# caojiezhang/CiaoSR

Hardware: AMD Instinct MI355X
Metric: HR Mpix/s (RDN-CiaoSR x4, LocalImplicitSR forward_test) (higher is better)
Workload: dtype f32; 1 GPU; C3: RDN-CiaoSR (c64b16) x4, LR 1356x2040 -> 5424x8160 (DIV2K-shaped 2K LR), tiled inference: 117 tiles of 192x192 (overlap 32), random-init weights, fp32; scale=4, tiles=117, parallelism=tile-shard x1

## Files before the change

### ciaosr_amd/_lib.py

```python
import ctypes as C
import os

_HERE = os.path.dirname(os.path.abspath(__file__))
LIB_PATH = os.environ.get('CIAOSR_HIP_LIB') or os.path.join(_HERE, 'csrc', 'libciaosr_hip.so')
MAX_LAYERS = 8

ACT_NONE, ACT_RELU, ACT_PRELU, ACT_GELU, ACT_SIN, ACT_COS = 0, 1, 2, 3, 4, 5


class CiaoSRHipError(RuntimeError):
    pass


class MlpT(C.Structure):
    _fields_ = [('n_layers', C.c_int), ('act', C.c_int), ('in_dim', C.c_int), ('width', C.c_int * MAX_LAYERS),
                ('weight', C.c_void_p * MAX_LAYERS), ('ld', C.c_int * MAX_LAYERS),
                ('bias', C.c_void_p * MAX_LAYERS), ('frag', C.c_void_p * MAX_LAYERS),
                ('frag16', C.c_void_p * MAX_LAYERS), ('frag16_lo', C.c_void_p * MAX_LAYERS)]


class HeadWeightsT(C.Structure):
    _fields_ = [('channels', C.c_int), ('nonlocal_channels', C.c_int), ('nonlocal_max_scale', C.c_int), ('local_size', C.c_int),
                ('no_unfold', C.c_int),
                ('softmax_scale', C.c_float), ('q', MlpT), ('k', MlpT), ('v', MlpT), ('k_out_wino', C.c_void_p), ('k_out_wino4', C.c_void_p),
                ('chain16', C.c_void_p), ('chain16_pairs', C.c_void_p)]


class HeadSceneT(C.Structure):
    _fields_ = [(n, C.c_int) for n in ('magic', 'H', 'W', 'C', 'Cn', 'D', 'Dv', 'J', 'q_plan', 'precision', 'route',
                                       'off_u', 'off_tk', 'off_tv', 'off_g', 'total')]


class CsAttnWeightsT(C.Structure):
    _fields_ = [('channels', C.c_int), ('scale', C.c_int),
                ('w_match1', C.c_void_p), ('b_match1', C.c_void_p), ('slope_match1', C.c_float),
                ('w_match2', C.c_void_p), ('b_match2', C.c_void_p), ('slope_match2', C.c_float),
                ('w_assembly', C.c_void_p), ('b_assembly', C.c_void_p), ('slope_assembly', C.c_float),
                ('w_down', C.c_void_p), ('b_down', C.c_void_p), ('w_down_masked', C.c_void_p),
                ('escape_nan', C.c_float), ('softmax_scale', C.c_float)]


class OptionsT(C.Structure):
    _fields_ = [('head_route', C.c_int), ('csa_composed_min', C.c_int), ('dense_min_tiles', C.c_int),
                ('scatter_small_max', C.c_int), ('kv_rows', C.c_int), ('decode_rows', C.c_int), ('bf16_single', C.c_int),
                ('dense_direct', C.c_int), ('csa_scores_gemm', C.c_int), ('csa_attn_tile128', C.c_int), ('query_grid_w', C.c_int), ('f16_pairs', C.c_int),
                ('csa_attn_v16', C.c_int), ('edsr_resident', C.c_int), ('swin_h16', C.c_int), ('csa_block_mb', C.c_int)]


HEAD_STAGED, HEAD_NO_LOGIT_TABLE, HEAD_TABLE_GEMM, HEAD_WIDE_WG, HEAD_TABLE_WINO2, HEAD_NO_CHAIN, HEAD_NO_DECODE_CHAIN = 1, 2, 4, 8, 16, 32, 64


class ConvT(C.Structure):
    _fields_ = [('weight', C.c_void_p), ('bias', C.c_void_p), ('cin', C.c_int), ('cout', C.c_int), ('ksize', C.c_int),
                ('frag16', C.c_void_p), ('frag16_lo', C.c_void_p), ('frag', C.c_void_p), ('frag_wino', C.c_void_p),
                ('frag_wino4', C.c_void_p)]


class RdnWeightsT(C.Structure):
    _fields_ = [('mid_channels', C.c_int), ('growth', C.c_int), ('num_blocks', C.c_int), ('num_layers', C.c_int),
                ('sfe1', ConvT), ('sfe2', ConvT), ('gff0', ConvT), ('gff1', ConvT),
                ('dense', C.POINTER(ConvT)), ('lff', C.POINTER(ConvT)),
                ('scatter_weight', C.POINTER(C.c_void_p)), ('scatter_bias', C.c_void_p),
                ('scatter_frag', C.POINTER(C.c_void_p))]


class SwinBlockT(C.Structure):
    _fields_ = [(n, C.c_void_p) for n in ('ln1_w', 'ln1_b', 'qkv_w', 'qkv_b', 'bias', 'proj_w', 'proj_b', 'ln2_w', 'ln2_b',
                                           'fc1_w', 'fc1_b', 'fc2_w', 'fc2_b')] + [('shift', C.c_int), ('mask', C.c_void_p)] + \
               [(n, C.c_void_p) for n in ('qkv_w16', 'proj_w16', 'fc1_w16', 'fc2_w16')]


class SwinirWeightsT(C.Structure):
    _fields_ = [('embed_dim', C.c_int), ('num_heads', C.c_int), ('window_size', C.c_int), ('hidden', C.c_int),
                ('num_groups', C.c_int), ('depth', C.c_int), ('conv_first', ConvT), ('conv_after_body', ConvT),
                ('pe_norm_w', C.c_void_p), ('pe_norm_b', C.c_void_p), ('norm_w', C.c_void_p), ('norm_b', C.c_void_p),
                ('blocks', C.POINTER(SwinBlockT)), ('group_conv', C.POINTER(ConvT))]


class EdsrWeightsT(C.Structure):
    _fields_ = [('mid_channels', C.c_int), ('num_blocks', C.c_int), ('res_scale', C.c_float),
                ('conv_first', ConvT), ('conv_after_body', ConvT),
                ('conv1', C.POINTER(ConvT)), ('conv2', C.POINTER(ConvT))]


_P, _I, _F, _S = C.c_void_p, C.c_int, C.c_float, C.c_size_t
_O = C.POINTER(OptionsT)

SIGNATURES = {
    'ciaosr_version': (_I, []),
    'ciaosr_error_string': (C.c_char_p, [_I]),
    'ciaosr_sizeof': (_S, [C.c_char_p]),
    'ciaosr_prof_enable': (_I, [_I]),
    'ciaosr_prof_filter': (_I, [C.c_char_p]),
    'ciaosr_prof_reset': (_I, []),
    'ciaosr_prof_collect': (_I, []),
    'ciaosr_prof_get': (_I, [C.c_char_p, C.POINTER(C.c_double), C.POINTER(C.c_long)]),
    'ciaosr_prof_names': (_I, [C.c_char_p, _I]),
    'ciaosr_nchw_to_hwc_f32': (_I, [_P, _P, _I, _I, _I, _I, _P]),
    'ciaosr_hwc_to_nchw_f32': (_I, [_P, _I, _P, _I, _I, _I, _P]),
    'ciaosr_gemm_f32': (_I, [_P, _I, _P, _I, _I, _P, _I, _P, _I, _I, _I, _F, _I, _F, _P]),
    'ciaosr_patch_rows_f32': (_I, [_P, _I, _I, _I, _I, _I, _I, _I, _I, _I, _P, _I, _I, _F, _P]),
    'ciaosr_cs_attn_workspace_bytes': (_S, [_I, _I, _I]),
    'ciaosr_cs_attn_workspace_bytes_scale': (_S, [_I, _I, _I, _I]),
    'ciaosr_cs_attn_workspace_bytes_opt': (_S, [_I, _I, _I, _I, _O]),
    'ciaosr_cs_attn_block_rows': (_I, [_I, _I, _I, _I, _I, _O]),
    'ciaosr_cs_attn_f32': (_I, [_P, _I, _I, _I, C.POINTER(CsAttnWeightsT), _P, _I, _O, _P, _S, _P]),
    'ciaosr_cs_attn_bf16': (_I, [_P, _I, _I, _I, C.POINTER(CsAttnWeightsT), _P, _I, _O, _P, _S, _P]),
    'ciaosr_make_coord_cell_f32': (_I, [_P, _P, _I, _I, _P]),
    'ciaosr_make_coord_cell_window_f32': (_I, [_P, _P, _I, _I, _I, _I, _I, _I, C.POINTER(_I), _P]),
    'ciaosr_fragment_floats': (_S, [_I, _I]),
    'ciaosr_pack_fragments_f32': (_I, [_P, _I, _I, _I, _P, _P]),
    'ciaosr_cs_attn_f16': (_I, [_P, _I, _I, _I, C.POINTER(CsAttnWeightsT), _P, _I, _O, _P, _S, _P]),
    'ciaosr_fragment_bf16_bytes': (_S, [_I, _I]),
    'ciaosr_fragment_f16_bytes': (_S, [_I, _I]),
    'ciaosr_pack_fragments_f16': (_I, [_P, _I, _I, _I, _P, _P]),
    'ciaosr_pack_fragments_bf16': (_I, [_P, _I, _I, _I, _P, _P]),
    'ciaosr_pack_fragments_bf16_lo': (_I, [_P, _I, _I, _I, _P, _P]),
    'ciaosr_pack_fragments_f16_lo': (_I, [_P, _I, _I, _I, _P, _P]),
    'ciaosr_pack_fragments_bf16_pair': (_I, [_P, _I, _I, _I, _P, _P, _P]),
    'ciaosr_pack_fragments_f16_pair': (_I, [_P, _I, _I, _I, _P, _P, _P]),
    'ciaosr_pack_conv3x3_f32': (_I, [_P, _S, _S, _S, _S, _I, _I, _P, _P, _P, _P]),
    'ciaosr_head_chain_bytes': (_S, [C.POINTER(HeadWeightsT), _I]),
    'ciaosr_pack_head_chain_bf16': (_I, [C.POINTER(HeadWeightsT), _I, _P, _P]),
    'ciaosr_pack_head_chain_f16': (_I, [C.POINTER(HeadWeightsT), _I, _P, _P]),
    'ciaosr_head_indices_f32': (_I, [_P, _P, _I, _I, _I, _I, _I, _P, _P, _P, _P]),
    'ciaosr_local_attention_f32': (_I, [_P, _I, _I, _I, _P, _P, _P, _I, _P, _I, _P, _I, _I, _I, _F, _P]),
    'ciaosr_local_attention_bf16': (_I, [_P, _I, _I, _I, _P, _P, _P, _I, _P, _I, _P, _I, _I, _I, _F, _P]),
    'ciaosr_local_attention_f16': (_I, [_P, _I, _I, _I, _P, _P, _P, _I, _P, _I, _P, _I, _I, _I, _F, _P]),
    'ciaosr_gather_rows_f32': (_I, [_P, _I, _I, _I, _P, _P, _I, _I, _I, _I, _I, _P, _I, _P, _I, _P, _I, _P, _P, _P]),
    'ciaosr_mlp_workspace_bytes': (_S, [C.POINTER(MlpT), _I]),
    'ciaosr_mlp_forward_f32': (_I, [_P, _I, C.POINTER(MlpT), _I, _I, _P, _I, _P, _S, _P]),
    'ciaosr_mlp_workspace_bytes_16': (_S, [C.POINTER(MlpT), _I]),
    'ciaosr_mlp_forward_bf16': (_I, [_P, _I, C.POINTER(MlpT), _I, _P, _I, _P, _S, _P]),
    'ciaosr_mlp_forward_f16': (_I, [_P, _I, C.POINTER(MlpT), _I, _P, _I, _P, _S, _P]),
    'ciaosr_decode_residual_f32': (_I, [_P, _I, _I, _P, _I, _P, _P, _P, _I, _I, _I, _P, _P]),
    'ciaosr_head_workspace_bytes': (_S, [_I, _I, C.POINTER(HeadWeightsT), _I]),
    'ciaosr_head_workspace_bytes_opt': (_S, [_I, _I, C.POINTER(HeadWeightsT), _I, _O]),
    'ciaosr_head_forward_f32': (_I, [_P, _I, _I, C.POINTER(HeadWeightsT), C.POINTER(CsAttnWeightsT), _P, _P, _P,
                                     _I, _I, _P, _O, _P, _S, _P]),
    'ciaosr_head_forward_bf16': (_I, [_P, _I, _I, C.POINTER(HeadWeightsT), C.POINTER(CsAttnWeightsT), _P, _P, _P,
                                      _I, _I, _P, _O, _P, _S, _P]),
    'ciaosr_head_forward_f16': (_I, [_P, _I, _I, C.POINTER(HeadWeightsT), C.POINTER(CsAttnWeightsT), _P, _P, _P,
                                      _I, _I, _P, _O, _P, _S, _P]),
    'ciaosr_head_route_code': (_I, [_I, _I, C.POINTER(HeadWeightsT), _I, _I, _O]),
    'ciaosr_head_scene_bytes': (_S, [_I, _I, C.POINTER(HeadWeightsT), _I, _O]),
    'ciaosr_head_prepare_workspace_bytes': (_S, [_I, _I, C.POINTER(HeadWeightsT), _I, _O]),
    'ciaosr_head_query_workspace_bytes': (_S, [C.POINTER(HeadSceneT), C.POINTER(HeadWeightsT), _I, _O]),
    'ciaosr_head_query_flag_offset': (_I, [C.POINTER(HeadSceneT), C.POINTER(HeadWeightsT), _I, _O, C.POINTER(_S)]),
    **{'ciaosr_head_prepare_' + sfx: (_I, [_P, _I, _I, C.POINTER(HeadWeightsT), C.POINTER(CsAttnWeightsT), _I, _O, _P, _S,
                                          C.POINTER(HeadSceneT), _P, _S, _P]) for sfx in ('f32', 'bf16', 'f16')},
    **{'ciaosr_head_query_' + sfx: (_I, [_P, _S, C.POINTER(HeadSceneT), C.POINTER(HeadWeightsT), _P, _P, _P, _I, _I, _P, _O, _P, _S, _P])
       for sfx in ('f32', 'bf16', 'f16')},
    'ciaosr_rdn_workspace_bytes': (_S, [_I, _I, C.POINTER(RdnWeightsT)]),
    'ciaosr_rdn_forward_f32': (_I, [_P, _I, _I, C.POINTER(RdnWeightsT), _P, _O, _P, _S, _P]),
    'ciaosr_rdn_forward_bf16': (_I, [_P, _I, _I, C.POINTER(RdnWeightsT), _P, _O, _P, _S, _P]),
    'ciaosr_rdn_forward_f16': (_I, [_P, _I, _I, C.POINTER(RdnWeightsT), _P, _O, _P, _S, _P]),
    'ciaosr_rdn_workspace_bytes_batch': (_S, [_I, _I, _I, C.POINTER(RdnWeightsT)]),
    'ciaosr_rdn_forward_batch_f32': (_I, [_P, _I, _I, _I, C.POINTER(RdnWeightsT), _P, _O, _P, _S, _P]),
    'ciaosr_rdn_forward_batch_bf16': (_I, [_P, _I, _I, _I, C.POINTER(RdnWeightsT), _P, _O, _P, _S, _P]),
    'ciaosr_rdn_forward_batch_f16': (_I, [_P, _I, _I, _I, C.POINTER(RdnWeightsT), _P, _O, _P, _S, _P]),
    'ciaosr_edsr_workspace_bytes': (_S, [_I, _I, C.POINTER(EdsrWeightsT)]),
    'ciaosr_edsr_forward_f32': (_I, [_P, _I, _I, C.POINTER(EdsrWeightsT), _P, _P, _S, _P]),
    'ciaosr_edsr_workspace_bytes_batch': (_S, [_I, _I, _I, C.POINTER(EdsrWeightsT), _O]),
    'ciaosr_edsr_route_code': (_I, [_I, _I, _I, C.POINTER(EdsrWeightsT), _O]),
    'ciaosr_edsr_forward_batch_f32': (_I, [_P, _I, _I, _I, C.POINTER(EdsrWeightsT), _P, _O, _P, _S, _P]),
    'ciaosr_swinir_workspace_bytes': (_S, [_I, _I, C.POINTER(SwinirWeightsT)]),
    'ciaosr_swinir_forward_f32': (_I, [_P, _I, _I, C.POINTER(SwinirWeightsT), _P, _P, _S, _P]),
    'ciaosr_swinir_workspace_bytes_batch_f16': (_S, [_I, _I, _I, C.POINTER(SwinirWeightsT)]),
    'ciaosr_swinir_forward_batch_f16': (_I, [_P, _I, _I, _I, C.POINTER(SwinirWeightsT), _P, _O, _P, _S, _P]),
    'ciaosr_normalize_f32': (_I, [_P, _P, _I, _I, C.POINTER(_F), C.POINTER(_F), _P]),
    'ciaosr_denorm_clamp_f32': (_I, [_P, _P, _I, _I, C.POINTER(_F), C.POINTER(_F), _P]),
    'ciaosr_tile_blend_f32': (_I, [_P, _P, _I, _I, _P, _I, _I, _I, _I, _P]),
    'ciaosr_tile_finalize_f32': (_I, [_P, _P, _P, _I, _I, _P]),
    'ciaosr_view_block_queries': (_I, []),
    'ciaosr_view_workspace_bytes': (_S, [_I, _I, _I]),
    'ciaosr_view_coord_cell_f32': (_I, [_P, _P, C.POINTER(C.c_double), _I, _I, C.POINTER(_I), _P]),
    'ciaosr_view_count_i32': (_I, [C.POINTER(C.c_double), _I, _I, _P, _I, _P, _P, _S, _P]),
    'ciaosr_view_count_many_max_views': (_I, []),
    'ciaosr_view_many_workspace_bytes': (_S, [C.POINTER(_I), _I, _I]),
    'ciaosr_view_many_workspace_offset': (_S, [C.POINTER(_I), _I, _I, _I]),
# ... 57 lines not shown
```

### ciaosr_amd/csrc/dense_wino4_f32.hip

```cpp
#include "ops.h"
#include <type_traits>

namespace ciaosr {

typedef float f32x16 __attribute__((ext_vector_type(16)));
typedef float f32x4 __attribute__((ext_vector_type(4)));
typedef float f32x2 __attribute__((ext_vector_type(2)));
typedef int i32x4 __attribute__((ext_vector_type(4)));

constexpr int W4TH = 16, W4TW = 32;
constexpr int W4PH = W4TH + 2, W4PW = W4TW + 2;
constexpr int W4NP = W4PH * W4PW;
constexpr int W4PIECES = (2 * W4NP + 63) / 64;
constexpr int W4PATCH = W4PIECES * 1024;
constexpr int W4VROW = 32;
constexpr int W4VPOS = 32 * W4VROW;
constexpr int W4V = 36 * W4VPOS;
constexpr int W4V0 = 2 * W4PATCH;
constexpr size_t kWino4Xch = 4 * 8 * 4 * 64 * 16;
constexpr size_t kWino4Loop = 2 * (size_t)W4PATCH + 2 * (size_t)W4V;
constexpr size_t kWino4Lds = kWino4Loop > kWino4Xch ? kWino4Loop : kWino4Xch;
constexpr unsigned kOobW4 = 0xFFFFFFF0u;

struct DenseWino4P {
    float* x; int ldx;
    unsigned x_bytes;
    int H, W, tiles_x;
    int groups;
    const float4* wf;
    int nj; long pos_stride;
    const float* bias;
    int col_out;
    float* out; unsigned out_bytes;
    int ld_out; unsigned out_img_bytes;
    unsigned wf_block_bytes;
};

struct W4Slot { int vfrag, window, w2, dma, wnext; };
constexpr W4Slot w4_slot_plan(int r3, int slot) {
    W4Slot s = {-1, -1, -1, -1, -1};
    if (r3 < 2 && slot % 4 == 0) s.vfrag = slot / 4;
    if (r3 < 2 && slot % 2 == 1) s.window = 12 * r3 + slot / 2;
    if (r3 == 0 && slot < 6) s.w2 = slot;
    if (r3 == 0 && slot >= 6 && slot % 4 == 2) s.dma = (slot - 6) / 4;
    if (r3 == 1 && slot % 4 == 2) s.wnext = slot / 4;
    if (r3 == 2 && slot < 18) {
        if (slot % 3 == 2) s.wnext = 6 + slot / 3;
        else s.window = 24 + 2 * (slot / 3) + slot % 3;
    }
    return s;
}

#define W4_BT(x0, x1, x2, x3, x4, x5, y0, y1, y2, y3, y4, y5)                          \
    do {                                                                               \
        const float t1_ = __builtin_fmaf(-4.f, x2, x4), t2_ = __builtin_fmaf(-4.f, x1, x3); \
        const float t3_ = x4 - x2, t4_ = x3 - x1;                                      \
        y0 = __builtin_fmaf(4.f, x0, __builtin_fmaf(-5.f, x2, x4));                   \
        y1 = t1_ + t2_;                                                                \
        y2 = t1_ - t2_;                                                                \
        y3 = __builtin_fmaf(2.f, t4_, t3_);                                            \
        y4 = __builtin_fmaf(-2.f, t4_, t3_);                                           \
        y5 = __builtin_fmaf(4.f, x1, __builtin_fmaf(-5.f, x3, x5));                   \
    } while (0)

#ifdef CIAOSR_PROBE
__device__ unsigned long long g_w4probe[1024 * 8];
#define W4PROBE(slot) do { if (threadIdx.x == 0 && blockIdx.y == 0 && blockIdx.x < 1024) g_w4probe[blockIdx.x * 8 + (slot)] = __builtin_readcyclecounter(); } while (0)
#define W4PROBE_ADD(slot, t0) do { w4acc##slot += __builtin_readcyclecounter() - (t0); } while (0)
#else
#define W4PROBE(slot) do { } while (0)
#define W4PROBE_ADD(slot, t0) do { } while (0)
#endif

template <bool TABLE>
__global__ __launch_bounds__(256) void dense_wino4_f32_kernel(DenseWino4P p) {
    extern __shared__ __attribute__((aligned(16))) unsigned char lds4[];
    W4PROBE(0);
#ifdef CIAOSR_PROBE
    unsigned long long w4acc5 = 0, w4acc6 = 0;
#endif
    const int t = threadIdx.x, lane = t & 63, w = __builtin_amdgcn_readfirstlane(t >> 6), li = lane & 31, lh = lane >> 5;
    const int nt = w & 1, h = w >> 1;
    const int ty0 = (blockIdx.x / p.tiles_x) * W4TH, tx0 = (blockIdx.x % p.tiles_x) * W4TW;
    const int img = blockIdx.y;
    const unsigned img_off = (unsigned)((size_t)img * p.H * p.W * p.ldx * 4);
    const unsigned lds0 = (unsigned)(size_t)(__attribute__((address_space(3))) unsigned char*)lds4;

    constexpr int W4DS = W4PIECES / 4;
    unsigned goff[W4DS];
#pragma unroll
    for (int s = 0; s < W4DS; ++s) {
        const int qs = 64 * (w + 4 * s) + lane;
        const int q = qs ^ (((qs >> 3) & 3) << 1);
        const int P = q >> 1, half = q & 1;
        const int py = P / W4PW, px = P - py * W4PW;
        const int gy = ty0 - 1 + py, gx = tx0 - 1 + px;
        const bool ok = P < W4NP && gy >= 0 && gy < p.H && gx >= 0 && gx < p.W;
        goff[s] = ok ? (img_off + (unsigned)(gy * p.W + gx) * (unsigned)p.ldx * 4u + (unsigned)half * 16u) : kOobW4;
    }
    const int rot = p.groups > 1 ? (int)(blockIdx.x % (unsigned)p.groups) : 0;
    auto phys = [&](int g) -> int { const int x = g + rot; return x >= p.groups ? x - p.groups : x; };
    const i32x4 desc = {(int)(unsigned)(size_t)p.x, (int)(((size_t)p.x >> 32) & 0xFFFFu), (int)p.x_bytes, 0x00020000};
    const int N = 8 * p.groups;
    auto step_ch = [&](int n) -> int { return 64 * phys(n >> 3) + 8 * (n & 7); };
    auto dma_patch = [&](int n) {
        const unsigned soff = __builtin_amdgcn_readfirstlane((unsigned)step_ch(n) * 4u);
#pragma unroll
        for (int s = 0; s < W4DS; ++s) {
            const unsigned dst = __builtin_amdgcn_readfirstlane(lds0 + (unsigned)((n & 1) * W4PATCH) + 1024u * (unsigned)(w + 4 * s));
            unsigned keep;
            asm volatile("s_mov_b32 %0, m0\n\ts_mov_b32 m0, %2\n\ts_nop 0\n\tbuffer_load_dwordx4 %1, %3, %4 offen lds\n\ts_mov_b32 m0, %0"
                         : "=&s"(keep) : "v"(goff[s]), "s"(dst), "s"(desc), "s"(soff) : "memory");
        }
    };

    const int tch = t & 7, ttile = t >> 3;
    const int ttyw = ttile >> 3, ttxw = ttile & 7;
    int ty[4][4];
    {
        const int P0 = 4 * W4PW * ttyw + 4 * ttxw;
        const int k0 = (P0 >> 2) & 3;
        const int tbase = 32 * P0 + 16 * (tch >> 2) + 4 * (tch & 3);
#pragma unroll
        for (int m = 0; m < 4; ++m)
#pragma unroll
            for (int c = 0; c < 4; ++c) ty[m][c] = tbase + 32 * (m ^ ((k0 + c) & 3));
    }
    const int tvoff = ((2 * ttile + (tch >> 2)) ^ ((ttile >> 3) & 1)) * 16 + (tch & 3) * 4;

    const i32x4 wdesc = {(int)(unsigned)(size_t)p.wf, (int)(((size_t)p.wf >> 32) & 0xFFFFu), (int)0xFFFFFFFFu, 0x00020000};
    const unsigned lane16 = (unsigned)lane * 16u;
    const unsigned pos_bytes = (unsigned)p.pos_stride * 16u;
    auto wload = [&](f32x4& dst, int pp, int n) __attribute__((always_inline)) {
        const unsigned so = __builtin_amdgcn_readfirstlane((unsigned)(18 * h + pp) * pos_bytes + (unsigned)(nt * p.nj + (step_ch(n) >> 3)) * 1024u +
                                                           (TABLE ? (unsigned)blockIdx.z * p.wf_block_bytes : 0u));
        asm volatile("buffer_load_dwordx4 %0, %1, %2, %3 offen" : "=v"(dst) : "v"(lane16), "s"(wdesc), "s"(so) : "memory");
    };

    dma_patch(0);
    if (N > 1) dma_patch(1);
    f32x4 wr[18];
#pragma unroll
    for (int pp = 0; pp < 12; ++pp) wload(wr[pp], pp, 0);
    __builtin_amdgcn_sched_barrier(0);
    f32x16 acc[18];
#pragma unroll
    for (int pp = 0; pp < 18; ++pp)
#pragma unroll
        for (int e = 0; e < 16; ++e) acc[pp][e] = 0.f;
    asm volatile("s_waitcnt vmcnt(12)" ::: "memory");
    __builtin_amdgcn_s_barrier();
    __builtin_amdgcn_sched_barrier(0);

    W4PROBE(1);
    float dn[36];
    auto patch_value = [&](int n, int o36) __attribute__((always_inline)) -> float {
        const int a = o36 / 6, b = o36 - 6 * a, o = W4PW * a + b;
        return *reinterpret_cast<const float*>(lds4 + (n & 1) * W4PATCH + ty[o & 3][(o >> 2) & 3] + 32 * (o & ~3));
    };
#pragma unroll
    for (int o36 = 0; o36 < 36; ++o36) dn[o36] = patch_value(0, o36);
    const int vfo = ((2 * li + lh) ^ ((li >> 3) & 1)) * 16;
#pragma unroll 1
    for (int n = 0; n < N; ++n) {
#ifdef CIAOSR_PROBE
        const unsigned long long tstep = __builtin_readcyclecounter();
#endif
        {
            unsigned char* vb = lds4 + W4V0 + (n & 1) * W4V + tvoff;
            float d[6][6];
#pragma unroll
            for (int a = 0; a < 6; ++a)
#pragma unroll
                for (int b = 0; b < 6; ++b) d[a][b] = dn[6 * a + b];
            float r[6][6];
#pragma unroll
            for (int bp = 0; bp < 3; ++bp) {
                f32x2 x[6], y[6];
#pragma unroll
                for (int a = 0; a < 6; ++a) x[a] = f32x2{d[a][2 * bp], d[a][2 * bp + 1]};
                const f32x2 t1 = __builtin_elementwise_fma(f32x2{-4.f, -4.f}, x[2], x[4]), t2 = __builtin_elementwise_fma(f32x2{-4.f, -4.f}, x[1], x[3]);
                const f32x2 t3 = x[4] - x[2], t4 = x[3] - x[1];
                y[0] = __builtin_elementwise_fma(f32x2{4.f, 4.f}, x[0], __builtin_elementwise_fma(f32x2{-5.f, -5.f}, x[2], x[4]));
                y[1] = t1 + t2;
                y[2] = t1 - t2;
                y[3] = __builtin_elementwise_fma(f32x2{2.f, 2.f}, t4, t3);
                y[4] = __builtin_elementwise_fma(f32x2{-2.f, -2.f}, t4, t3);
                y[5] = __builtin_elementwise_fma(f32x2{4.f, 4.f}, x[1], __builtin_elementwise_fma(f32x2{-5.f, -5.f}, x[3], x[5]));
#pragma unroll
                for (int i = 0; i < 6; ++i) { r[i][2 * bp] = y[i][0]; r[i][2 * bp + 1] = y[i][1]; }
            }
#pragma unroll
            for (int i = 0; i < 6; ++i) {
                float v0, v1, v2, v3, v4, v5;
                W4_BT(r[i][0], r[i][1], r[i][2], r[i][3], r[i][4], r[i][5], v0, v1, v2, v3, v4, v5);
                *reinterpret_cast<float*>(vb + (6 * i + 0) * W4VPOS) = v0;
                *reinterpret_cast<float*>(vb + (6 * i + 1) * W4VPOS) = v1;
                *reinterpret_cast<float*>(vb + (6 * i + 2) * W4VPOS) = v2;
                *reinterpret_cast<float*>(vb + (6 * i + 3) * W4VPOS) = v3;
                *reinterpret_cast<float*>(vb + (6 * i + 4) * W4VPOS) = v4;
                *reinterpret_cast<float*>(vb + (6 * i + 5) * W4VPOS) = v5;
            }
        }
        asm volatile("s_waitcnt vmcnt(12)" ::: "memory");
        W4PROBE_ADD(5, tstep);
        __syncthreads();
        W4PROBE_ADD(6, tstep);
        __builtin_amdgcn_sched_barrier(0);
        {
            const unsigned char* vb = lds4 + W4V0 + (n & 1) * W4V + 18 * h * W4VPOS + vfo;
            float4 vf[2][6];
#pragma unroll
            for (int j = 0; j < 6; ++j) vf[0][j] = *reinterpret_cast<const float4*>(vb + j * W4VPOS);
            const int n1 = n + 1 < N ? n + 1 : N - 1, n2 = n + 2 < N ? n + 2 : N - 1;
            const unsigned dsoff = __builtin_amdgcn_readfirstlane((unsigned)step_ch(n2) * 4u);
            const unsigned ddst = lds0 + (unsigned)((n & 1) * W4PATCH) + 1024u * (unsigned)w;
            auto mma = [&](int pp, float a, float bq) __attribute__((always_inline)) {
                if (pp < 16) acc[pp] = __builtin_amdgcn_mfma_f32_32x32x2f32(a, bq, acc[pp], 0, 0, 0);
                else asm volatile("v_mfma_f32_32x32x2_f32 %0, %1, %2, %0" : "+v"(acc[pp]) : "v"(a), "v"(bq));
            };
#pragma unroll
            for (int r3 = 0; r3 < 3; ++r3) {
                if (r3 == 0) asm volatile("s_waitcnt vmcnt(6)" ::: "memory");
                else asm volatile("s_waitcnt vmcnt(11)" ::: "memory");
                __builtin_amdgcn_sched_barrier(0);
#pragma unroll
                for (int slot = 0; slot < 24; ++slot) {
                    const int c = slot / 6, j = slot % 6, pp = 6 * r3 + j;
                    const f32x4 wv = wr[pp];
                    const float4 bv = vf[r3 & 1][j];
                    mma(pp, c == 0 ? wv.x : c == 1 ? wv.y : c == 2 ? wv.z : wv.w, c == 0 ? bv.x : c == 1 ? bv.y : c == 2 ? bv.z : bv.w);
                    const W4Slot sp = w4_slot_plan(r3, slot);
                    if (sp.vfrag >= 0)
                        vf[(r3 + 1) & 1][sp.vfrag] = *reinterpret_cast<const float4*>(vb + (6 * (r3 + 1) + sp.vfrag) * W4VPOS);
                    if (sp.window >= 0) dn[sp.window] = patch_value(n + 1, sp.window);
                    if (sp.w2 >= 0) wload(wr[12 + sp.w2], 12 + sp.w2, n);
                    if (sp.dma >= 0) {
                        const unsigned dst = __builtin_amdgcn_readfirstlane(ddst + 4096u * (unsigned)sp.dma);
                        unsigned keep;
                        asm volatile("s_mov_b32 %0, m0\n\ts_mov_b32 m0, %2\n\ts_nop 0\n\tbuffer_load_dwordx4 %1, %3, %4 offen lds\n\ts_mov_b32 m0, %0"
                                     : "=&s"(keep) : "v"(goff[sp.dma]), "s"(dst), "s"(desc), "s"(dsoff) : "memory");
                    }
                    if (sp.wnext >= 0) wload(wr[sp.wnext], sp.wnext, n1);
                    __builtin_amdgcn_sched_barrier(0);
                }
            }
            if (n + 1 == N) asm volatile("s_waitcnt vmcnt(0)" ::: "memory");
        }
    }
    W4PROBE(2);
#ifdef CIAOSR_PROBE
    if (threadIdx.x == 0 && blockIdx.y == 0 && blockIdx.x < 1024) { g_w4probe[blockIdx.x * 8 + 5] = w4acc5; g_w4probe[blockIdx.x * 8 + 6] = w4acc6; }
#endif
    __syncthreads();

    float4* xch = reinterpret_cast<float4*>(lds4);
    f32x4 own[4][2][4];
    auto out_pass = [&](auto qc) __attribute__((always_inline)) {
        constexpr int q = decltype(qc)::value;
        auto grp = [&](const f32x16& v) __attribute__((always_inline)) -> f32x4 { return __builtin_shufflevector(v, v, 4 * q, 4 * q + 1, 4 * q + 2, 4 * q + 3); };
        f32x4 tt[3][4];
#pragma unroll
        for (int r = 0; r < 3; ++r) {
            const f32x4 m0 = grp(acc[6 * r]), m1 = grp(acc[6 * r + 1]), m2 = grp(acc[6 * r + 2]), m3 = grp(acc[6 * r + 3]), m4 = grp(acc[6 * r + 4]), m5 = grp(acc[6 * r + 5]);
            const f32x4 s1 = m1 + m2, d1 = m1 - m2, s2 = m3 + m4, d2 = m3 - m4;
            tt[r][0] = m0 + s1 + s2;
            tt[r][1] = d1 + 2.f * d2;
            tt[r][2] = s1 + 4.f * s2;
            tt[r][3] = d1 + 8.f * d2 + m5;
        }
#pragma unroll
        for (int x = 0; x < 4; ++x) {
            f32x4 keep0, keep1, send0, send1;
            if (h == 0) {
                const f32x4 d = tt[1][x] - tt[2][x], sm = tt[1][x] + tt[2][x];
                keep0 = tt[0][x] + sm; keep1 = d; send0 = sm; send1 = d;
            } else {
                const f32x4 sm = tt[0][x] + tt[1][x], d = tt[0][x] - tt[1][x];
                send0 = sm; send1 = 2.f * d; keep0 = 4.f * sm; keep1 = 8.f * d + tt[2][x];
            }
            own[q][0][x] = keep0;
            own[q][1][x] = keep1;
            xch[((w * 8 + x) * 4 + q) * 64 + lane] = make_float4(send0[0], send0[1], send0[2], send0[3]);
            xch[((w * 8 + 4 + x) * 4 + q) * 64 + lane] = make_float4(send1[0], send1[1], send1[2], send1[3]);
        }
    };
    out_pass(std::integral_constant<int, 0>{});
    out_pass(std::integral_constant<int, 1>{});
    out_pass(std::integral_constant<int, 2>{});
    out_pass(std::integral_constant<int, 3>{});
    __syncthreads();
    W4PROBE(3);
    {
        const int pw = w ^ 2;
        const __amdgpu_buffer_rsrc_t ors = TABLE ? __builtin_amdgcn_make_buffer_rsrc(p.out, 0, p.out_bytes, 0x00020000)
                                                 : __builtin_amdgcn_make_buffer_rsrc(p.x, 0, p.x_bytes, 0x00020000);
        const unsigned o_img = TABLE ? (unsigned)img * p.out_img_bytes : img_off;
        const unsigned o_ld = TABLE ? (unsigned)p.ld_out : (unsigned)p.ldx;
        const int o_col = TABLE ? 64 * (int)blockIdx.z : p.col_out;
        float4 bias4[4];
#pragma unroll
        for (int q = 0; q < 4; ++q) bias4[q] = TABLE ? make_float4(0.f, 0.f, 0.f, 0.f) : *reinterpret_cast<const float4*>(p.bias + 32 * nt + 8 * q + 4 * lh);
        float4 o[2][4];
#pragma unroll
        for (int q = 0; q < 4; ++q) o[0][q] = xch[((pw * 8 + 0) * 4 + q) * 64 + lane];
#pragma unroll
        for (int it = 0; it < 8; ++it) {
            const int yy = it >> 2, x = it & 3;
            if (it + 1 < 8) {
#pragma unroll
                for (int q = 0; q < 4; ++q) o[(it + 1) & 1][q] = xch[((pw * 8 + it + 1) * 4 + q) * 64 + lane];
            }
            unsigned char* tb = reinterpret_cast<unsigned char*>(xch + ((pw * 8 + it) * 4) * 64);
#pragma unroll
            for (int q = 0; q < 4; ++q) {
                const float4 ov = o[it & 1][q];
                float4 v;
                if (TABLE) {
                    v.x = own[q][yy][x][0] + ov.x; v.y = own[q][yy][x][1] + ov.y; v.z = own[q][yy][x][2] + ov.z; v.w = own[q][yy][x][3] + ov.w;
                } else {
                    v.x = fmaxf(own[q][yy][x][0] + ov.x + bias4[q].x, 0.f);
                    v.y = fmaxf(own[q][yy][x][1] + ov.y + bias4[q].y, 0.f);
                    v.z = fmaxf(own[q][yy][x][2] + ov.z + bias4[q].z, 0.f);
                    v.w = fmaxf(own[q][yy][x][3] + ov.w + bias4[q].w, 0.f);
                }
                *reinterpret_cast<float4*>(tb + li * 128 + (((2 * q + lh) ^ (li & 7)) << 4)) = v;
            }
            wave_lds_sync();
            const int sr = lane >> 3, sc = lane & 7;
            const int xx = tx0 + 4 * sr + x;
#pragma unroll
            for (int j = 0; j < 4; ++j) {
                const int tl = 8 * j + sr;
                const float4 v = *reinterpret_cast<const float4*>(tb + tl * 128 + ((sc ^ (tl & 7)) << 4));
                const int y = ty0 + 4 * j + 2 * h + yy;
                const bool ok = y < p.H && xx < p.W;
                const unsigned pix = o_img + (unsigned)(y * p.W + xx) * o_ld * 4u + (unsigned)(o_col + 32 * nt + 4 * sc) * 4u;
                i32x4 iv;
                iv.x = __float_as_int(v.x); iv.y = __float_as_int(v.y); iv.z = __float_as_int(v.z); iv.w = __float_as_int(v.w);
                __builtin_amdgcn_raw_buffer_store_b128(iv, ors, (int)(ok ? pix : kOobW4), 0, 0);
            }
            __builtin_amdgcn_sched_barrier(0);
        }
    }
    W4PROBE(4);
#ifdef CIAOSR_PROBE
    asm volatile("s_waitcnt vmcnt(0)" ::: "memory");
    W4PROBE(7);
#endif
}

int dense_wino4_tiles(int H, int W) { return ceil_div(H, W4TH) * ceil_div(W, W4TW); }

int dense_layer_wino4_f32(float* X, int ldx, int H, int W, int l, const float* frag_wino4, const float* bias, int n_img, hipStream_t s) {
    CIAOSR_CHECK_ARG(X && frag_wino4 && bias && (ldx & 3) == 0 && aligned16(X) && aligned16(frag_wino4) && aligned16(bias));
    const size_t x_bytes = (size_t)n_img * H * W * ldx * 4;
    CIAOSR_CHECK_ARG(n_img >= 1 && n_img <= 65535 && x_bytes < 0xFFFFFF00ull);
    DenseWino4P p;
    p.x = X; p.ldx = ldx; p.x_bytes = (unsigned)x_bytes;
    p.H = H; p.W = W; p.tiles_x = ceil_div(W, W4TW);
    p.groups = l + 1;
    p.wf = reinterpret_cast<const float4*>(frag_wino4);
    p.nj = 64 * (l + 1) / 8;
    p.pos_stride = (long)2 * p.nj * 64;
    p.bias = bias;
    p.col_out = 64 * (l + 1);
    CIAOSR_CHECK_ARG((size_t)36 * p.pos_stride * 16 < 0xFFFFFF00ull);
    p.out = nullptr; p.out_bytes = 0; p.ld_out = 0; p.out_img_bytes = 0; p.wf_block_bytes = 0;
    CIAOSR_BIG_LDS(dense_wino4_f32_kernel<false>, kWino4Lds);
    ProfScope prof("enc_dense_wino4", s);
    hipLaunchKernelGGL(dense_wino4_f32_kernel<false>, dim3(dense_wino4_tiles(H, W), n_img), dim3(256), kWino4Lds, s, p);
    return launch_status("dense_wino4_f32");
}

int wino4_table_f32(const float* Pi, int H, int W, const float* frag_wino4, int n_blk, float* out, int ldg, hipStream_t s) {
    CIAOSR_CHECK_ARG(Pi && frag_wino4 && out && n_blk >= 1 && (ldg & 3) == 0 && aligned16(Pi) && aligned16(frag_wino4) && aligned16(out));
    const size_t in_bytes = (size_t)9 * H * W * 64 * 4, out_bytes = (size_t)9 * H * W * ldg * 4;
    CIAOSR_CHECK_ARG(in_bytes < 0xFFFFFF00ull && out_bytes < 0xFFFFFF00ull);
    DenseWino4P p;
    p.x = const_cast<float*>(Pi); p.ldx = 64; p.x_bytes = (unsigned)in_bytes;
    p.H = H; p.W = W; p.tiles_x = ceil_div(W, W4TW);
    p.groups = 1;
    p.wf = reinterpret_cast<const float4*>(frag_wino4);
    p.nj = 8;
    p.pos_stride = (long)2 * n_blk * p.nj * 64;
    p.wf_block_bytes = 2u * 8u * 1024u;
    p.bias = nullptr; p.col_out = 0;
    p.out = out; p.out_bytes = (unsigned)out_bytes; p.ld_out = 9 * ldg; p.out_img_bytes = (unsigned)ldg * 4u;
    CIAOSR_CHECK_ARG((size_t)36 * p.pos_stride * 16 < 0xFFFFFF00ull);
    CIAOSR_BIG_LDS(dense_wino4_f32_kernel<true>, kWino4Lds);
    ProfScope prof("head_logit_table_w4", s);
    hipLaunchKernelGGL(dense_wino4_f32_kernel<true>, dim3(dense_wino4_tiles(H, W), 9, n_blk), dim3(256), kWino4Lds, s, p);
    return launch_status("wino4_table_f32");
}

}

#ifdef CIAOSR_PROBE
extern "C" int ciaosr_debug_probe_w4_read(unsigned long long* host, int n_words) {
    return hipMemcpyFromSymbol(host, HIP_SYMBOL(ciaosr::g_w4probe), (size_t)n_words * 8) == hipSuccess ? 0 : -1;
}
#endif
```

### include/ciaosr_hip.h

```cpp
#ifndef CIAOSR_HIP_H
#define CIAOSR_HIP_H

#include <stddef.h>

#ifdef __cplusplus
extern "C" {
#endif

#define CIAOSR_OK 0
#define CIAOSR_ERR_BAD_ARG (-1)
#define CIAOSR_ERR_LAUNCH (-2)
#define CIAOSR_ERR_UNSUPPORTED (-3)
#define CIAOSR_ERR_WORKSPACE (-4)

#define CIAOSR_ACT_NONE 0
#define CIAOSR_ACT_RELU 1
#define CIAOSR_ACT_PRELU 2
#define CIAOSR_ACT_GELU 3
#define CIAOSR_ACT_SIN 4
#define CIAOSR_ACT_COS 5

#define CIAOSR_MAX_LAYERS 8

int ciaosr_version(void);
const char* ciaosr_error_string(int code);
size_t ciaosr_sizeof(const char* type_name );

int ciaosr_prof_enable(int on);
int ciaosr_prof_filter(const char* kernel );
int ciaosr_prof_reset(void);
int ciaosr_prof_collect(void);
int ciaosr_prof_get(const char* kernel, double* total_ms , long* launches );
int ciaosr_prof_names(char* buf , int buflen);

#define CIAOSR_HEAD_STAGED 1
#define CIAOSR_HEAD_TABLE_GEMM 4
#define CIAOSR_HEAD_NO_LOGIT_TABLE 2
#define CIAOSR_HEAD_WIDE_WG 8
#define CIAOSR_HEAD_TABLE_WINO2 16
#define CIAOSR_HEAD_NO_CHAIN 32
#define CIAOSR_HEAD_NO_DECODE_CHAIN 64
typedef struct ciaosr_options {
    int head_route;
    int csa_composed_min;
    int dense_min_tiles;
    int scatter_small_max;
    int kv_rows;
    int decode_rows;
    int bf16_single;
    int dense_direct;
    int csa_scores_gemm;
    int csa_attn_tile128;
    int query_grid_w;
    int f16_pairs;
    int csa_attn_v16;
    int edsr_resident;
    int swin_h16;
    int csa_block_mb;
} ciaosr_options_t;

int ciaosr_nchw_to_hwc_f32(const float* src, float* dst, int C, int H, int W, int ld_dst, void* stream);
int ciaosr_hwc_to_nchw_f32(const float* src, int ld_src, float* dst, int C, int H, int W, void* stream);

int ciaosr_gemm_f32(const float* A, int lda, const float* B, int ldb, int b_is_kn, float* C, int ldc,
                    const float* bias, int M, int N, int K, float alpha, int act, float slope,
                    void* stream);

int ciaosr_patch_rows_f32(const float* src_hwc, int ld_src, int Hs, int Ws, int Cs, int ksize, int stride,
                          int pad, int OH, int OW, float* out, int ld_out, int l2_normalize,
                          float norm_floor, void* stream);

typedef struct ciaosr_csattn_weights {
    int channels;
    int scale;
    const float* w_match1;
    const float* b_match1;
    float slope_match1;
    const float* w_match2;
    const float* b_match2;
    float slope_match2;
    const float* w_assembly;
    const float* b_assembly;
    float slope_assembly;
    const float* w_down;
    const float* b_down;
    const float* w_down_masked;
    float escape_nan;
    float softmax_scale;
} ciaosr_csattn_weights_t;

size_t ciaosr_cs_attn_workspace_bytes(int H, int W, int C);
size_t ciaosr_cs_attn_workspace_bytes_scale(int H, int W, int C, int scale);
size_t ciaosr_cs_attn_workspace_bytes_opt(int H, int W, int C, int scale, const ciaosr_options_t* opt );
int ciaosr_cs_attn_block_rows(int H, int W, int C, int scale, int precision, const ciaosr_options_t* opt );
int ciaosr_cs_attn_f32(const float* feat_hwc, int ld_feat, int H, int W, const ciaosr_csattn_weights_t* w,
                       float* out, int ld_out, const ciaosr_options_t* opt , void* workspace,
                       size_t workspace_bytes, void* stream);
int ciaosr_cs_attn_bf16(const float* feat_hwc, int ld_feat, int H, int W, const ciaosr_csattn_weights_t* w,
                        float* out, int ld_out, const ciaosr_options_t* opt , void* workspace,
                        size_t workspace_bytes, void* stream);
int ciaosr_cs_attn_f16(const float* feat_hwc, int ld_feat, int H, int W, const ciaosr_csattn_weights_t* w,
                       float* out, int ld_out, const ciaosr_options_t* opt , void* workspace,
                       size_t workspace_bytes, void* stream);

typedef struct ciaosr_mlp {
    int n_layers;
    int act;
    int in_dim;
    int width[CIAOSR_MAX_LAYERS];
    const float* weight[CIAOSR_MAX_LAYERS];
    int ld[CIAOSR_MAX_LAYERS];
    const float* bias[CIAOSR_MAX_LAYERS];
    const float* frag[CIAOSR_MAX_LAYERS];
    const void* frag16[CIAOSR_MAX_LAYERS];
    const void* frag16_lo[CIAOSR_MAX_LAYERS];
} ciaosr_mlp_t;
// ... 265 lines not shown
```

Baseline: 11.98 Mpix/s.

## Make Winograd-4 dense kernel persistent with a grid-stride loop over tile items

Converts the F(4,3) Winograd dense/table kernel from one workgroup per tile into a persistent kernel. The grid is capped at the CU count and each workgroup loops over flattened (block, image, tile) items. Per-item indices are computed as scalars, and the channel-group rotation is now based on the tile instead of blockIdx. It also adds explicit accvgpr reads and sched barriers in the output transform to steer register allocation. The aim is to cut launch/tail wave cost and amortise setup, at the risk of load imbalance and an extra __syncthreads per item.

Result: no change. 12.01 Mpix/s, median of 6 (+0.2%).

```diff
diff --git a/ciaosr_amd/_lib.py b/ciaosr_amd/_lib.py
--- a/ciaosr_amd/_lib.py
+++ b/ciaosr_amd/_lib.py
@@ -96,6 +96,7 @@
     'ciaosr_prof_collect': (_I, []),
     'ciaosr_prof_get': (_I, [C.c_char_p, C.POINTER(C.c_double), C.POINTER(C.c_long)]),
     'ciaosr_prof_names': (_I, [C.c_char_p, _I]),
+    'ciaosr_dev_wino4_grid_cap': (_I, [_I]),
     'ciaosr_nchw_to_hwc_f32': (_I, [_P, _P, _I, _I, _I, _I, _P]),
     'ciaosr_hwc_to_nchw_f32': (_I, [_P, _I, _P, _I, _I, _I, _P]),
     'ciaosr_gemm_f32': (_I, [_P, _I, _P, _I, _I, _P, _I, _P, _I, _I, _I, _F, _I, _F, _P]),
diff --git a/ciaosr_amd/csrc/dense_wino4_f32.hip b/ciaosr_amd/csrc/dense_wino4_f32.hip
--- a/ciaosr_amd/csrc/dense_wino4_f32.hip
+++ b/ciaosr_amd/csrc/dense_wino4_f32.hip
@@ -26,6 +26,7 @@
     float* x; int ldx;
     unsigned x_bytes;
     int H, W, tiles_x;
+    int tiles, n_img, items;
     int groups;
     const float4* wf;
     int nj; long pos_stride;
@@ -64,8 +65,9 @@
     } while (0)
 
 #ifdef CIAOSR_PROBE
-__device__ unsigned long long g_w4probe[1024 * 8];
-#define W4PROBE(slot) do { if (threadIdx.x == 0 && blockIdx.y == 0 && blockIdx.x < 1024) g_w4probe[blockIdx.x * 8 + (slot)] = __builtin_readcyclecounter(); } while (0)
+__device__ unsigned long long g_w4probe[1024 * 16];
+#define W4PROBE_ON (threadIdx.x == 0 && w4pid < 1024)
+#define W4PROBE(slot) do { if (W4PROBE_ON) g_w4probe[w4pid * 16 + (slot)] = __builtin_readcyclecounter(); } while (0)
 #define W4PROBE_ADD(slot, t0) do { w4acc##slot += __builtin_readcyclecounter() - (t0); } while (0)
 #else
 #define W4PROBE(slot) do { } while (0)
@@ -75,18 +77,40 @@
 template <bool TABLE>
 __global__ __launch_bounds__(256) void dense_wino4_f32_kernel(DenseWino4P p) {
     extern __shared__ __attribute__((aligned(16))) unsigned char lds4[];
+    const int w = __builtin_amdgcn_readfirstlane((int)threadIdx.x >> 6);
+    const int nt = w & 1, h = w >> 1;
+    auto thread_index = []() __attribute__((always_inline)) -> int { int x = (int)threadIdx.x; asm volatile("" : "+v"(x)); return x; };
+    const unsigned lds0 = (unsigned)(size_t)(__attribute__((address_space(3))) unsigned char*)lds4;
+    constexpr int W4DS = W4PIECES / 4;
+    const i32x4 desc = {(int)(unsigned)(size_t)p.x, (int)(((size_t)p.x >> 32) & 0xFFFFu), (int)p.x_bytes, 0x00020000};
+    const int N = 8 * p.groups;
+
+    const i32x4 wdesc = {(int)(unsigned)(size_t)p.wf, (int)(((size_t)p.wf >> 32) & 0xFFFFu), (int)0xFFFFFFFFu, 0x00020000};
+    const unsigned pos_bytes = (unsigned)p.pos_stride * 16u;
+
+#pragma unroll 1
+    for (int item = (int)blockIdx.x; item < p.items; item += (int)gridDim.x) {
+#ifdef CIAOSR_PROBE
+    const int w4pid = item;
+    unsigned long long w4acc5 = 0, w4acc6 = 0;
+    if (W4PROBE_ON) {
+        g_w4probe[w4pid * 16 + 8] = ((unsigned long long)__builtin_amdgcn_s_getreg(63508) << 32) | __builtin_amdgcn_s_getreg(63492);
+        g_w4probe[w4pid * 16 + 9] = __builtin_amdgcn_s_memrealtime();
+    }
+#endif
     W4PROBE(0);
-#ifdef CIAOSR_PROBE
-    unsigned long long w4acc5 = 0, w4acc6 = 0;
-#endif
-    const int t = threadIdx.x, lane = t & 63, w = __builtin_amdgcn_readfirstlane(t >> 6), li = lane & 31, lh = lane >> 5;
-    const int nt = w & 1, h = w >> 1;
-    const int ty0 = (blockIdx.x / p.tiles_x) * W4TH, tx0 = (blockIdx.x % p.tiles_x) * W4TW;
-    const int img = blockIdx.y;
+    auto scalar = [](int x) __attribute__((always_inline)) -> int { x = __builtin_amdgcn_readfirstlane(x); asm("" : "+s"(x)); return x; };
+    const int rest = scalar(item / p.tiles), tile = item - rest * p.tiles;
+    const int zblk = TABLE ? scalar(rest / p.n_img) : 0, img = TABLE ? rest - zblk * p.n_img : rest;
+    const int tyi = scalar(tile / p.tiles_x);
+    const int ty0 = tyi * W4TH, tx0 = (tile - tyi * p.tiles_x) * W4TW;
     const unsigned img_off = (unsigned)((size_t)img * p.H * p.W * p.ldx * 4);
-    const unsigned lds0 = (unsigned)(size_t)(__attribute__((address_space(3))) unsigned char*)lds4;
-
-    constexpr int W4DS = W4PIECES / 4;
+    f32x16 acc[18];
+    {
+    const int t = thread_index(), lane = t & 63, li = lane & 31, lh = lane >> 5;
+    const unsigned lane16 = (unsigned)lane * 16u;
+    const int vfo = ((2 * li + lh) ^ ((li >> 3) & 1)) * 16;
+
     unsigned goff[W4DS];
 #pragma unroll
     for (int s = 0; s < W4DS; ++s) {
@@ -98,22 +122,6 @@
         const bool ok = P < W4NP && gy >= 0 && gy < p.H && gx >= 0 && gx < p.W;
         goff[s] = ok ? (img_off + (unsigned)(gy * p.W + gx) * (unsigned)p.ldx * 4u + (unsigned)half * 16u) : kOobW4;
     }
-    const int rot = p.groups > 1 ? (int)(blockIdx.x % (unsigned)p.groups) : 0;
-    auto phys = [&](int g) -> int { const int x = g + rot; return x >= p.groups ? x - p.groups : x; };
-    const i32x4 desc = {(int)(unsigned)(size_t)p.x, (int)(((size_t)p.x >> 32) & 0xFFFFu), (int)p.x_bytes, 0x00020000};
-    const int N = 8 * p.groups;
-    auto step_ch = [&](int n) -> int { return 64 * phys(n >> 3) + 8 * (n & 7); };
-    auto dma_patch = [&](int n) {
-        const unsigned soff = __builtin_amdgcn_readfirstlane((unsigned)step_ch(n) * 4u);
-#pragma unroll
-        for (int s = 0; s < W4DS; ++s) {
-            const unsigned dst = __builtin_amdgcn_readfirstlane(lds0 + (unsigned)((n & 1) * W4PATCH) + 1024u * (unsigned)(w + 4 * s));
-            unsigned keep;
-            asm volatile("s_mov_b32 %0, m0\n\ts_mov_b32 m0, %2\n\ts_nop 0\n\tbuffer_load_dwordx4 %1, %3, %4 offen lds\n\ts_mov_b32 m0, %0"
-                         : "=&s"(keep) : "v"(goff[s]), "s"(dst), "s"(desc), "s"(soff) : "memory");
-        }
-    };
-
     const int tch = t & 7, ttile = t >> 3;
     const int ttyw = ttile >> 3, ttxw = ttile & 7;
     int ty[4][4];
@@ -128,12 +136,22 @@
     }
     const int tvoff = ((2 * ttile + (tch >> 2)) ^ ((ttile >> 3) & 1)) * 16 + (tch & 3) * 4;
 
-    const i32x4 wdesc = {(int)(unsigned)(size_t)p.wf, (int)(((size_t)p.wf >> 32) & 0xFFFFu), (int)0xFFFFFFFFu, 0x00020000};
-    const unsigned lane16 = (unsigned)lane * 16u;
-    const unsigned pos_bytes = (unsigned)p.pos_stride * 16u;
+    const int rot = p.groups > 1 ? scalar((int)((unsigned)tile % (unsigned)p.groups)) : 0;
+    auto phys = [&](int g) -> int { const int x = g + rot; return x >= p.groups ? x - p.groups : x; };
+    auto step_ch = [&](int n) -> int { return 64 * phys(n >> 3) + 8 * (n & 7); };
+    auto dma_patch = [&](int n) {
+        const unsigned soff = __builtin_amdgcn_readfirstlane((unsigned)step_ch(n) * 4u);
+#pragma unroll
+        for (int s = 0; s < W4DS; ++s) {
+            const unsigned dst = __builtin_amdgcn_readfirstlane(lds0 + (unsigned)((n & 1) * W4PATCH) + 1024u * (unsigned)(w + 4 * s));
+            unsigned keep;
+            asm volatile("s_mov_b32 %0, m0\n\ts_mov_b32 m0, %2\n\ts_nop 0\n\tbuffer_load_dwordx4 %1, %3, %4 offen lds\n\ts_mov_b32 m0, %0"
+                         : "=&s"(keep) : "v"(goff[s]), "s"(dst), "s"(desc), "s"(soff) : "memory");
+        }
+    };
     auto wload = [&](f32x4& dst, int pp, int n) __attribute__((always_inline)) {
         const unsigned so = __builtin_amdgcn_readfirstlane((unsigned)(18 * h + pp) * pos_bytes + (unsigned)(nt * p.nj + (step_ch(n) >> 3)) * 1024u +
-                                                           (TABLE ? (unsigned)blockIdx.z * p.wf_block_bytes : 0u));
+                                                           (TABLE ? (unsigned)zblk * p.wf_block_bytes : 0u));
         asm volatile("buffer_load_dwordx4 %0, %1, %2, %3 offen" : "=v"(dst) : "v"(lane16), "s"(wdesc), "s"(so) : "memory");
     };
 
@@ -143,7 +161,6 @@
 #pragma unroll
     for (int pp = 0; pp < 12; ++pp) wload(wr[pp], pp, 0);
     __builtin_amdgcn_sched_barrier(0);
-    f32x16 acc[18];
 #pragma unroll
     for (int pp = 0; pp < 18; ++pp)
 #pragma unroll
@@ -160,7 +177,6 @@
     };
 #pragma unroll
     for (int o36 = 0; o36 < 36; ++o36) dn[o36] = patch_value(0, o36);
-    const int vfo = ((2 * li + lh) ^ ((li >> 3) & 1)) * 16;
 #pragma unroll 1
     for (int n = 0; n < N; ++n) {
 #ifdef CIAOSR_PROBE
@@ -248,26 +264,38 @@
             if (n + 1 == N) asm volatile("s_waitcnt vmcnt(0)" ::: "memory");
         }
     }
+    }
     W4PROBE(2);
 #ifdef CIAOSR_PROBE
-    if (threadIdx.x == 0 && blockIdx.y == 0 && blockIdx.x < 1024) { g_w4probe[blockIdx.x * 8 + 5] = w4acc5; g_w4probe[blockIdx.x * 8 + 6] = w4acc6; }
+    if (W4PROBE_ON) { g_w4probe[w4pid * 16 + 5] = w4acc5; g_w4probe[w4pid * 16 + 6] = w4acc6; }
 #endif
     __syncthreads();
+    __builtin_amdgcn_sched_barrier(0);
 
     float4* xch = reinterpret_cast<float4*>(lds4);
+    const int lane = thread_index() & 63, li = lane & 31, lh = lane >> 5;
     f32x4 own[4][2][4];
     auto out_pass = [&](auto qc) __attribute__((always_inline)) {
         constexpr int q = decltype(qc)::value;
-        auto grp = [&](const f32x16& v) __attribute__((always_inline)) -> f32x4 { return __builtin_shufflevector(v, v, 4 * q, 4 * q + 1, 4 * q + 2, 4 * q + 3); };
+        auto grp = [&](int pp) __attribute__((always_inline)) -> f32x4 {
+            if (pp >= 16) return __builtin_shufflevector(acc[pp], acc[pp], 4 * q, 4 * q + 1, 4 * q + 2, 4 * q + 3);
+            float g0, g1, g2, g3;
+            asm("v_accvgpr_read_b32 %0, %1" : "=v"(g0) : "a"(acc[pp][4 * q]));
+            asm("v_accvgpr_read_b32 %0, %1" : "=v"(g1) : "a"(acc[pp][4 * q + 1]));
+            asm("v_accvgpr_read_b32 %0, %1" : "=v"(g2) : "a"(acc[pp][4 * q + 2]));
+            asm("v_accvgpr_read_b32 %0, %1" : "=v"(g3) : "a"(acc[pp][4 * q + 3]));
+            return f32x4{g0, g1, g2, g3};
+        };
         f32x4 tt[3][4];
 #pragma unroll
         for (int r = 0; r < 3; ++r) {
-            const f32x4 m0 = grp(acc[6 * r]), m1 = grp(acc[6 * r + 1]), m2 = grp(acc[6 * r + 2]), m3 = grp(acc[6 * r + 3]), m4 = grp(acc[6 * r + 4]), m5 = grp(acc[6 * r + 5]);
+            const f32x4 m0 = grp(6 * r), m1 = grp(6 * r + 1), m2 = grp(6 * r + 2), m3 = grp(6 * r + 3), m4 = grp(6 * r + 4), m5 = grp(6 * r + 5);
             const f32x4 s1 = m1 + m2, d1 = m1 - m2, s2 = m3 + m4, d2 = m3 - m4;
             tt[r][0] = m0 + s1 + s2;
             tt[r][1] = d1 + 2.f * d2;
             tt[r][2] = s1 + 4.f * s2;
             tt[r][3] = d1 + 8.f * d2 + m5;
+            __builtin_amdgcn_sched_barrier(0);
         }
 #pragma unroll
         for (int x = 0; x < 4; ++x) {
@@ -283,11 +311,15 @@
             own[q][1][x] = keep1;
             xch[((w * 8 + x) * 4 + q) * 64 + lane] = make_float4(send0[0], send0[1], send0[2], send0[3]);
             xch[((w * 8 + 4 + x) * 4 + q) * 64 + lane] = make_float4(send1[0], send1[1], send1[2], send1[3]);
+            __builtin_amdgcn_sched_barrier(0);
         }
     };
     out_pass(std::integral_constant<int, 0>{});
+    __builtin_amdgcn_sched_barrier(0);
     out_pass(std::integral_constant<int, 1>{});
+    __builtin_amdgcn_sched_barrier(0);
     out_pass(std::integral_constant<int, 2>{});
+    __builtin_amdgcn_sched_barrier(0);
     out_pass(std::integral_constant<int, 3>{});
     __syncthreads();
     W4PROBE(3);
@@ -297,7 +329,7 @@
                                                  : __builtin_amdgcn_make_buffer_rsrc(p.x, 0, p.x_bytes, 0x00020000);
         const unsigned o_img = TABLE ? (unsigned)img * p.out_img_bytes : img_off;
         const unsigned o_ld = TABLE ? (unsigned)p.ld_out : (unsigned)p.ldx;
-        const int o_col = TABLE ? 64 * (int)blockIdx.z : p.col_out;
+        const int o_col = TABLE ? 64 * zblk : p.col_out;
         float4 bias4[4];
 #pragma unroll
         for (int q = 0; q < 4; ++q) bias4[q] = TABLE ? make_float4(0.f, 0.f, 0.f, 0.f) : *reinterpret_cast<const float4*>(p.bias + 32 * nt + 8 * q + 4 * lh);
@@ -315,14 +347,15 @@
 #pragma unroll
             for (int q = 0; q < 4; ++q) {
                 const float4 ov = o[it & 1][q];
+                const f32x4 kq = own[q][yy][x];
                 float4 v;
                 if (TABLE) {
-                    v.x = own[q][yy][x][0] + ov.x; v.y = own[q][yy][x][1] + ov.y; v.z = own[q][yy][x][2] + ov.z; v.w = own[q][yy][x][3] + ov.w;
+                    v.x = kq[0] + ov.x; v.y = kq[1] + ov.y; v.z = kq[2] + ov.z; v.w = kq[3] + ov.w;
                 } else {
-                    v.x = fmaxf(own[q][yy][x][0] + ov.x + bias4[q].x, 0.f);
-                    v.y = fmaxf(own[q][yy][x][1] + ov.y + bias4[q].y, 0.f);
-                    v.z = fmaxf(own[q][yy][x][2] + ov.z + bias4[q].z, 0.f);
-                    v.w = fmaxf(own[q][yy][x][3] + ov.w + bias4[q].w, 0.f);
+                    v.x = fmaxf(kq[0] + ov.x + bias4[q].x, 0.f);
+                    v.y = fmaxf(kq[1] + ov.y + bias4[q].y, 0.f);
+                    v.z = fmaxf(kq[2] + ov.z + bias4[q].z, 0.f);
+                    v.w = fmaxf(kq[3] + ov.w + bias4[q].w, 0.f);
                 }
                 *reinterpret_cast<float4*>(tb + li * 128 + (((2 * q + lh) ^ (li & 7)) << 4)) = v;
             }
@@ -347,10 +380,23 @@
 #ifdef CIAOSR_PROBE
     asm volatile("s_waitcnt vmcnt(0)" ::: "memory");
     W4PROBE(7);
-#endif
+    if (W4PROBE_ON) g_w4probe[w4pid * 16 + 10] = __builtin_amdgcn_s_memrealtime();
+#endif
+    __syncthreads();
+    }
 }
 
 int dense_wino4_tiles(int H, int W) { return ceil_div(H, W4TH) * ceil_div(W, W4TW); }
+
+static std::atomic<int> g_wino4_grid_cap{0};
+static int wino4_grid(long items) {
+    int dev = 0, cus = 256;
+    if (hipGetDevice(&dev) == hipSuccess) (void)hipDeviceGetAttribute(&cus, hipDeviceAttributeMultiprocessorCount, dev);
+    const int cap = g_wino4_grid_cap.load(std::memory_order_relaxed);
+    long g = cus > 0 ? cus : 256;
+    if (cap > 0 && cap < g) g = cap;
+    return (int)(items < g ? items : g);
+}
 
 int dense_layer_wino4_f32(float* X, int ldx, int H, int W, int l, const float* frag_wino4, const float* bias, int n_img, hipStream_t s) {
     CIAOSR_CHECK_ARG(X && frag_wino4 && bias && (ldx & 3) == 0 && aligned16(X) && aligned16(frag_wino4) && aligned16(bias));
@@ -359,6 +405,9 @@
     DenseWino4P p;
     p.x = X; p.ldx = ldx; p.x_bytes = (unsigned)x_bytes;
     p.H = H; p.W = W; p.tiles_x = ceil_div(W, W4TW);
+    p.tiles = dense_wino4_tiles(H, W); p.n_img = n_img;
+    CIAOSR_CHECK_ARG((long)p.tiles * n_img < 0x7FFF0000l);
+    p.items = p.tiles * n_img;
     p.groups = l + 1;
     p.wf = reinterpret_cast<const float4*>(frag_wino4);
     p.nj = 64 * (l + 1) / 8;
@@ -369,7 +418,7 @@
     p.out = nullptr; p.out_bytes = 0; p.ld_out = 0; p.out_img_bytes = 0; p.wf_block_bytes = 0;
     CIAOSR_BIG_LDS(dense_wino4_f32_kernel<false>, kWino4Lds);
     ProfScope prof("enc_dense_wino4", s);
-    hipLaunchKernelGGL(dense_wino4_f32_kernel<false>, dim3(dense_wino4_tiles(H, W), n_img), dim3(256), kWino4Lds, s, p);
+    hipLaunchKernelGGL(dense_wino4_f32_kernel<false>, dim3(wino4_grid(p.items)), dim3(256), kWino4Lds, s, p);
     return launch_status("dense_wino4_f32");
 }
 
@@ -380,6 +429,9 @@
     DenseWino4P p;
     p.x = const_cast<float*>(Pi); p.ldx = 64; p.x_bytes = (unsigned)in_bytes;
     p.H = H; p.W = W; p.tiles_x = ceil_div(W, W4TW);
+    p.tiles = dense_wino4_tiles(H, W); p.n_img = 9;
+    CIAOSR_CHECK_ARG((long)p.tiles * 9 * n_blk < 0x7FFF0000l);
+    p.items = p.tiles * 9 * n_blk;
     p.groups = 1;
     p.wf = reinterpret_cast<const float4*>(frag_wino4);
     p.nj = 8;
@@ -390,11 +442,13 @@
     CIAOSR_CHECK_ARG((size_t)36 * p.pos_stride * 16 < 0xFFFFFF00ull);
     CIAOSR_BIG_LDS(dense_wino4_f32_kernel<true>, kWino4Lds);
     ProfScope prof("head_logit_table_w4", s);
-    hipLaunchKernelGGL(dense_wino4_f32_kernel<true>, dim3(dense_wino4_tiles(H, W), 9, n_blk), dim3(256), kWino4Lds, s, p);
+    hipLaunchKernelGGL(dense_wino4_f32_kernel<true>, dim3(wino4_grid(p.items)), dim3(256), kWino4Lds, s, p);
     return launch_status("wino4_table_f32");
 }
 
 }
+
+extern "C" int ciaosr_dev_wino4_grid_cap(int cap) { return ciaosr::g_wino4_grid_cap.exchange(cap > 0 ? cap : 0); }
 
 #ifdef CIAOSR_PROBE
 extern "C" int ciaosr_debug_probe_w4_read(unsigned long long* host, int n_words) {
diff --git a/include/ciaosr_hip.h b/include/ciaosr_hip.h
--- a/include/ciaosr_hip.h
+++ b/include/ciaosr_hip.h
@@ -32,6 +32,8 @@
 int ciaosr_prof_collect(void);
 int ciaosr_prof_get(const char* kernel, double* total_ms , long* launches );
 int ciaosr_prof_names(char* buf , int buflen);
+
+int ciaosr_dev_wino4_grid_cap(int cap);
 
 #define CIAOSR_HEAD_STAGED 1
 #define CIAOSR_HEAD_TABLE_GEMM 4
```
